# maotian123/loc_lib

Hardware: NVIDIA B200
Metric: registered_points_per_sec (higher is better)
Workload: dtype f64

## Files before the change

loc_lib_b200/csrc/icp_pipeline.cuh:

```cuda
#pragma once
#include "device_utils.cuh"
#include "icp_point.cuh"
#include "knn_warp.cuh"

namespace locreg {

struct DevResult {
    int iters, updates, converged, degenerate;
    long long n_effective, n_inlier;
    double sum_sq_res;
    int pose_written, pad_;
};
static_assert(sizeof(DevResult) == 48, "DevResult must match locreg_result");

struct AlignState {
    double pose[7];
    DevResult res;
    int stop;
    int pad;
};

constexpr int kTile = 256;
constexpr unsigned int kNoNeighbour = kNoPos;

// ... 104 lines not shown
    if (threadIdx.x == 0) tile_begin[S] = carry;
}

__global__ void k_tile_table(BatchView bv, unsigned int n_tiles, TileRec* tiles) {
    const unsigned int t = blockIdx.x * blockDim.x + threadIdx.x;
    if (t >= n_tiles) return;
    bv.tiles = nullptr;
    const TileCoord c = locate_tile_thread(bv, t);
    TileRec r;
    r.scan = c.scan; r.first = c.first; r.count = c.valid ? c.count : 0u; r.valid = c.valid ? 1u : 0u;
    r.base = c.src_base; r.pad = 0;
    tiles[t] = r;
}

#ifndef LR_NN_MIN_BLOCKS
#define LR_NN_MIN_BLOCKS 6
#endif
constexpr int kNnSeeds = 1, kNnTwoPass = 2;
struct RingQueue {
    unsigned int* count;
    uint2* entries;
};

__device__ __forceinline__ void tile_queue_append(bool mine, unsigned int row, unsigned int scan, unsigned int* pending,
                                                  unsigned int* done, unsigned int* staged, const RingQueue& queue,
                                                  unsigned int* local_rows = nullptr, unsigned int* local_n = nullptr) {
    const unsigned int lane = threadIdx.x & 31, n_warps = blockDim.x >> 5;
#if defined(LR_APPEND_BARRIER)
    if (mine) staged[atomicAdd(pending, 1u)] = row;
    __syncthreads();
    if (threadIdx.x >= 32) return;
    (void)done; (void)n_warps;
    {
        const unsigned int n = *pending;
        if (n == 0u) return;
        if (local_rows != nullptr) {
            for (unsigned int i = lane; i < n; i += 32) local_rows[i] = staged[i];
            if (lane == 0) { *local_n = n; atomicAdd(queue.count, n); }
            return;
        }
        unsigned int base = 0;
        if (lane == 0) base = atomicAdd(queue.count, n);
        base = __shfl_sync(0xffffffffu, base, 0);
        for (unsigned int i = lane; i < n; i += 32) queue.entries[base + i] = make_uint2(staged[i], scan);
        return;
    }
#endif
    if (mine) staged[atomicAdd(pending, 1u)] = row;
    __syncwarp();
    unsigned int last = 0;
    if (lane == 0) {
        __threadfence_block();
        last = atomicAdd(done, 1u) == n_warps - 1 ? 1u : 0u;
        __threadfence_block();
    }
    if (!__shfl_sync(0xffffffffu, last, 0)) return;
    __syncwarp();
    const unsigned int n = *reinterpret_cast<volatile unsigned int*>(pending);
    if (n == 0u) return;
    if (local_rows != nullptr) {
        for (unsigned int i = lane; i < n; i += 32) local_rows[i] = reinterpret_cast<volatile unsigned int*>(staged)[i];
        if (lane == 0) { *local_n = n; atomicAdd(queue.count, n); }
        return;
    }
    unsigned int base = 0;
    if (lane == 0) base = atomicAdd(queue.count, n);
    base = __shfl_sync(0xffffffffu, base, 0);
    for (unsigned int i = lane; i < n; i += 32)
        queue.entries[base + i] = make_uint2(reinterpret_cast<volatile unsigned int*>(staged)[i], scan);
}

constexpr int kNnTrack = 4;
constexpr int kNnFirstTrack = 16;
constexpr int kNnFused = 8;
#ifndef LR_NN_TRACK_MIN_BLOCKS
#define LR_NN_TRACK_MIN_BLOCKS LR_NN_MIN_BLOCKS
#endif
template <int K, bool TRACKED>
__device__ __forceinline__ void icp_nn_tile(unsigned int tile, const VoxelMapView& map, const BatchView& bv,
                                            const AlignState* __restrict__ states, int ignore_stop, int mode,
                                            unsigned int* __restrict__ nn_pos, unsigned char* __restrict__ plane_valid, KnnTrack* track,
                                            const RingQueue& queue, unsigned int* local_rows = nullptr, unsigned int* local_n = nullptr) {
    __shared__ Pose T;
    const TileCoord tc = locate_tile(bv, tile);
    if (!tc.valid) return;
    const AlignState* st = states + tc.scan;
    if (st->stop && !ignore_stop) return;
    if (threadIdx.x == 0) pose_load(T, st->pose);
    __shared__ unsigned int blk_pending, blk_done, blk_scan;
    __shared__ unsigned int staged[kTile];
    __shared__ unsigned char scan_list[kTile];
    if (threadIdx.x == 0) { blk_pending = 0u; blk_done = 0u; blk_scan = 0u; }
// ... 49 lines not shown
        const float qx = static_cast<float>(wx), qy = static_cast<float>(wy), qz = static_cast<float>(wz);
        if (tracked) done = knn_query_fast_track<K>(map, qx, qy, qz, nn, seeds, tr);
        else done = knn_query_fast<K>(map, qx, qy, qz, nn, seeds, (mode & kNnTwoPass) != 0);
        same = done && (mode & kNnSeeds) != 0;
        same = same && knn_same_set<K>(seeds, nn.pos);
    }
    if (in_tile) {
#pragma unroll
        for (int j = 0; j < K; ++j) out[j] = nn.pos[j];
        if (plane_valid && !same) plane_valid[row] = 0;
        if (track) track[row] = tr;
    }
    tile_queue_append(!done, static_cast<unsigned int>(row), tc.scan, &blk_pending, &blk_done, staged, queue, local_rows, local_n);
}
template <int K, bool TRACKED>
__global__ void __launch_bounds__(kTile, TRACKED ? LR_NN_TRACK_MIN_BLOCKS : LR_NN_MIN_BLOCKS) k_icp_nn(VoxelMapView map, BatchView bv,
                                                                    const AlignState* __restrict__ states, int ignore_stop,
                                                                    int mode, unsigned int* __restrict__ nn_pos,
                                                                    unsigned char* __restrict__ plane_valid, KnnTrack* track,
                                                                    RingQueue queue) {
    icp_nn_tile<K, TRACKED>(blockIdx.x, map, bv, states, ignore_stop, mode, nn_pos, plane_valid, track, queue);
}

#ifndef LR_FINISH_MIN_BLOCKS
#define LR_FINISH_MIN_BLOCKS 8
#endif
template <int K>
__global__ void __launch_bounds__(128, LR_FINISH_MIN_BLOCKS) k_icp_nn_finish(VoxelMapView map, CoarseLevels coarse, BatchView bv,
                                                       const AlignState* __restrict__ states, unsigned int* __restrict__ nn_pos,
                                                       KnnTrack* track, RingQueue queue, unsigned int min_count, unsigned int max_count) {
    const unsigned int n = *queue.count;
    if (n < min_count || n >= max_count) return;
    const unsigned int lane = threadIdx.x & 31;
    while (true) {
        unsigned int base = 0;
        if (lane == 0) base = atomicAdd(queue.count + 1, 32u);
        base = __shfl_sync(0xffffffffu, base, 0);
        if (base >= n) break;
        const unsigned int e = base + lane;
        if (e >= n) continue;
        const uint2 q = queue.entries[e];
        const size_t src_idx = bv.offsets ? static_cast<size_t>(q.x) : static_cast<size_t>(q.x) - static_cast<size_t>(q.y) * bv.n_single;
        const float4 sp = bv.src[src_idx];
        Pose T;
        pose_load(T, states[q.y].pose);
        double wx, wy, wz;
// ... 28 lines not shown
    const float4 sp = bv.src[src_idx];
    Pose T;
    pose_load(T, states[q.y].pose);
    double wx, wy, wz;
    pose_apply(T, static_cast<double>(sp.x), static_cast<double>(sp.y), static_cast<double>(sp.z), wx, wy, wz);
    qx = static_cast<float>(wx); qy = static_cast<float>(wy); qz = static_cast<float>(wz);
}
__global__ void __launch_bounds__(256) k_queue_bin_count(BatchView bv, const AlignState* __restrict__ states, RingQueue queue,
                                                         unsigned int min_count, float inv_bin, unsigned int bucket_mask, int sub_bits,
                                                         unsigned int* __restrict__ bucket_of, unsigned int* hist) {
    const unsigned int n = *queue.count;
    if (n < min_count) return;
    for (unsigned int e = blockIdx.x * blockDim.x + threadIdx.x; e < n; e += gridDim.x * blockDim.x) {
        float qx, qy, qz;
        queue_entry_query(queue.entries[e], bv, states, qx, qy, qz);
        const int bx = cell_of(cell_coord_f(qx, inv_bin)), by = cell_of(cell_coord_f(qy, inv_bin)), bz = cell_of(cell_coord_f(qz, inv_bin));
        const unsigned long long key = pack_cell(bx >> sub_bits, by >> sub_bits, bz >> sub_bits);
        unsigned int mort = 0u;
        for (int j = 0; j < sub_bits; ++j)
            mort |= (((static_cast<unsigned int>(bx) >> j) & 1u) << (3 * j)) | (((static_cast<unsigned int>(by) >> j) & 1u) << (3 * j + 1)) |
                    (((static_cast<unsigned int>(bz) >> j) & 1u) << (3 * j + 2));
        const unsigned int b = ((hash_block(key) << (3 * sub_bits)) | mort) & bucket_mask;
        bucket_of[e] = b;
        atomicAdd(&hist[b], 1u);
    }
}
__global__ void __launch_bounds__(256) k_queue_bin_scatter(RingQueue queue, unsigned int min_count, const unsigned int* __restrict__ bucket_of,
                                                           unsigned int* cursor, uint2* __restrict__ sorted) {
    const unsigned int n = *queue.count;
    if (n < min_count) return;
    for (unsigned int e = blockIdx.x * blockDim.x + threadIdx.x; e < n; e += gridDim.x * blockDim.x)
        sorted[atomicAdd(&cursor[bucket_of[e]], 1u)] = queue.entries[e];
}

#ifndef LR_PYR_MIN_BLOCKS
#define LR_PYR_MIN_BLOCKS 8
#endif
#ifndef LR_PYR_REFILL
#define LR_PYR_REFILL 8
#endif
template <int K>
__global__ void __launch_bounds__(128, LR_PYR_MIN_BLOCKS) k_icp_nn_pyr(VoxelMapView map, const __grid_constant__ PyrView py, BatchView bv,
                                                    const AlignState* __restrict__ states, unsigned int* __restrict__ nn_pos,
                                                    KnnTrack* track, RingQueue queue, unsigned int min_count) {
    const unsigned int n = *queue.count;
    if (n < min_count) return;
    const unsigned int lane = threadIdx.x & 31;
    PyrWalk<K> w;
    unsigned long long todo[kPyrStack];
    constexpr int kFree = 4, kDead = 5;
    int st = kFree, bit = 0;
    bool exhausted = false;
    unsigned int row = 0;
    while (true) {
        const unsigned int b_node = __ballot_sync(0xffffffffu, st == kPyrNode), b_point = __ballot_sync(0xffffffffu, st == kPyrPoint),
// ... 540 lines not shown
```

loc_lib_b200/csrc/icp_staged.cuh:

```cuda
#pragma once
#include "icp_pipeline.cuh"

namespace locreg {

#ifndef LR_STAGE_CAP
#define LR_STAGE_CAP 2048
#endif
constexpr unsigned int kStageCap = LR_STAGE_CAP;
constexpr unsigned int kStageTab = 512;

template <int K>
struct KnnSel {
    float d[K];
    unsigned int p[K];
    float d6;
};
template <int K>
__device__ __forceinline__ void sel_init(KnnSel<K>& s) {
#pragma unroll
    for (int j = 0; j < K; ++j) { s.d[j] = INFINITY; s.p[j] = kNoPos; }
    s.d6 = INFINITY;
}
template <int K>
__device__ __forceinline__ void sel_push(KnnSel<K>& s, float d, unsigned int p) {
// ... 9 lines not shown
}
template <int K>
__device__ __forceinline__ bool sel_unambiguous(const KnnSel<K>& s) {
    bool ok = !(s.d[K - 1] == s.d6);
#pragma unroll
    for (int j = 0; j + 1 < K; ++j) ok = ok && !(s.d[j] == s.d[j + 1] && s.p[j + 1] != kNoPos);
    return ok;
}

LR_HD void knn_find_list_key(const VoxelMapView& m, unsigned long long key, unsigned int& beg, unsigned int& cnt) {
    unsigned int h = hash_block(key) & m.nbr_mask;
    beg = 0; cnt = 0;
    while (true) {
        const NbrSlot s = m.nbr_slots[h];
        if (s.key == key) { beg = s.start; cnt = s.count; return; }
        if (s.key == kEmptyKey) return;
        h = (h + 1) & m.nbr_mask;
    }
}

#ifndef LR_STAGED_MIN_BLOCKS
#define LR_STAGED_MIN_BLOCKS 4
#endif
template <int K, int MODE>
__global__ void __launch_bounds__(kTile, LR_STAGED_MIN_BLOCKS)
k_icp_nn_staged(VoxelMapView map, BatchView bv, const AlignState* __restrict__ states, int ignore_stop, unsigned int* __restrict__ nn_pos,
                unsigned char* __restrict__ plane_valid, KnnTrack* track, RingQueue queue) {
    __shared__ Pose T;
    __shared__ float4 s_cand[kStageCap];
    __shared__ unsigned long long s_key[kStageTab];
    __shared__ unsigned short s_slot_id[kStageTab];
    __shared__ unsigned long long s_lkey[kTile];
    __shared__ unsigned int s_beg[kTile], s_cnt[kTile];
    __shared__ unsigned int s_off[kTile + 1];
    __shared__ unsigned int s_nlists;
    __shared__ unsigned int blk_pending, blk_done;
    __shared__ unsigned int staged[kTile];
    const TileCoord tc = locate_tile(bv, blockIdx.x);
    if (!tc.valid) return;
    const AlignState* st = states + tc.scan;
    if (st->stop && !ignore_stop) return;
    if (threadIdx.x == 0) {
        pose_load(T, st->pose);
        blk_pending = 0u; blk_done = 0u; s_nlists = 0u;
    }
    for (unsigned int i = threadIdx.x; i < kStageTab; i += kTile) s_key[i] = kEmptyKey;
    const bool in_tile = threadIdx.x < tc.count;
    const unsigned int p = tc.first + (in_tile ? threadIdx.x : 0u);
    const float4 sp = bv.src[tc.src_base + p];
    const size_t row = static_cast<size_t>(tc.out_base + p);
    unsigned int* out = nn_pos + row * K;
    unsigned int seeds[K];
#pragma unroll
    for (int j = 0; j < K; ++j) seeds[j] = (MODE != 0 && in_tile) ? out[j] : kNoPos;
    __syncthreads();
    const bool valid = in_tile && finite3(sp.x, sp.y, sp.z) && map.n_pts != 0;
    float qx = 0.0f, qy = 0.0f, qz = 0.0f;
    KnnCellFrame c{};
    bool listed = false;
    unsigned int my_slot = 0;
    if (valid) {
        double wx, wy, wz;
        pose_apply(T, static_cast<double>(sp.x), static_cast<double>(sp.y), static_cast<double>(sp.z), wx, wy, wz);
        qx = static_cast<float>(wx); qy = static_cast<float>(wy); qz = static_cast<float>(wz);
        c = knn_frame(map, qx, qy, qz);
        listed = c.R0 == 1;
        if (listed) {
            const unsigned long long key = pack_cell(c.fx, c.fy, c.fz);
            unsigned int h = hash_block(key) & (kStageTab - 1);
            while (true) {
                const unsigned long long prev = atomicCAS(&s_key[h], kEmptyKey, key);
                if (prev == kEmptyKey) {
                    const unsigned int id = atomicAdd(&s_nlists, 1u);
                    s_slot_id[h] = static_cast<unsigned short>(id);
                    s_lkey[id] = key;
                    break;
                }
                if (prev == key) break;
                h = (h + 1) & (kStageTab - 1);
            }
            my_slot = h;
        }
    }
    KnnResult<K> res;
    knn_init(res);
    float4 sd[K];
// ... 92 lines not shown
        }
        if (sel_unambiguous(sel)) {
#pragma unroll
            for (int j = 0; j < K; ++j) { res.d2[j] = sel.d[j]; res.pos[j] = sel.p[j]; }
        } else {
            knn_init(res);
            knn_seed<K>(map, qx, qy, qz, seeds, res);
            sel.d6 = INFINITY;
            if (listed) {
                const float4* lst = off < kStageCap ? s_cand + off : map.pts + s_beg[id];
                for (unsigned int i = 0; i < cnt; ++i) {
                    const float4 p = lst[i];
                    knn_offer_track(map.pts, res, dis2_f32(qx, qy, qz, p.x, p.y, p.z), static_cast<unsigned int>(float_as_int(p.w)), sel.d6);
                }
            }
        }
        if (listed) {
            done = knn_list_final<K>(map, c, res);
            if (MODE == 2 && done) tr.margin = knn_track_margin<K>(map, c, res, sel.d6, qx, qy, qz);
        }
        same = done && MODE != 0;
        same = same && knn_same_set<K>(seeds, res.pos);
    }
    if (in_tile) {
#pragma unroll
        for (int j = 0; j < K; ++j) out[j] = res.pos[j];
        if (plane_valid && !same) plane_valid[row] = 0;
        if (track) track[row] = tr;
    }
    tile_queue_append(!done, static_cast<unsigned int>(row), tc.scan, &blk_pending, &blk_done, staged, queue);
}

}
```

loc_lib_b200/csrc/locreg.cu:

```cuda
#include "../../include/locreg.h"

#include <algorithm>
#include <cstdio>
#include <cstdlib>
#include <cstring>
#include <string>
#include <deque>
#include <vector>

#include "align_kernels.cuh"
#include "device_map.cuh"
#include "device_inc_ndt.cuh"
#include "device_ndt.cuh"
#include "filters.cuh"
#include "icp_fused.cuh"
#include "icp_staged.cuh"
#include "icp_persist.cuh"
#include "reloc_select.cuh"
#include "nccl_dyn.h"

#include <nvtx3/nvToolsExt.h>

using namespace locreg;

// ... 57 lines not shown
    std::vector<cudaStream_t> chunk_streams;
    std::vector<cudaEvent_t> chunk_done;
    cudaEvent_t loam_ev[2] = {nullptr, nullptr};
    DeviceVoxelMap icp_map;
    DeviceVoxelMap icp_coarse[kCoarseLevels];
    DeviceVoxelMap icp_mid;
    CoarseLevels coarse_views(int mid_shells = -1, int coarse_shells = -1) const {
        CoarseLevels c{};
        c.mid_shells_p1 = mid_shells + 1;
        c.coarse_shells_p1 = coarse_shells + 1;
        for (int l = 0; l < kCoarseLevels; ++l) c.lv[l] = icp_coarse[l].view();
        c.mid = icp_mid.view();
        c.pyr = icp_map.pyramid();
        c.pyr_mode = 0;
        return c;
    }
    DeviceNdtMap ndt_map;
    DeviceIncNdtMap inc_ndt_map;
    bool has_target = false;
    ncclComm_t comm = nullptr;
    int comm_rank = 0, comm_world = 1;
    DevBuf d_gather_pose, d_gather_res, d_bcast;
    DevBuf d_raw, d_src4, d_out, d_partials, d_state, d_acc, d_gate, d_nn, d_offsets, d_poses_in, d_poses_out, d_results,
        d_scores, d_misc, d_target, d_nnpos, d_tile_begin, d_tiles, d_states, d_ringq, d_ringc, d_sortq, d_sortb, d_sorth, d_rescanq, d_rescanc, d_loam, d_lmap_new, d_global, d_local, d_same, d_plane, d_pstat, d_track;
    DevBuf d_stage_keys, d_stage_slot, d_stage_idx, d_stage_poses, d_stage_scores, d_stage_rounds, d_stage_sel;
    size_t n_global = 0, global_stride = 0;
    struct KeyFrame { void* p = nullptr; size_t n = 0; };
    std::deque<KeyFrame> keyframes;
    DevBuf d_lmap, d_lmap_tmp;
    size_t n_lmap = 0, lmap_stride = 0;
    void clear_keyframes() {
        for (KeyFrame& k : keyframes) if (k.p) cudaFree(k.p);
        keyframes.clear();
        n_lmap = 0; lmap_stride = 0;
    }
    PinBuf h_in, h_out, h_small;
    double last_ms = 0;
    long long last_launches = 0;
    bool profile = false;
    std::vector<cudaEvent_t> prof_events;
    std::vector<int> prof_class;
    double prof_ms[4] = {0, 0, 0, 0};
    long long prof_launches[4] = {0, 0, 0, 0};
    std::vector<float> prof_trace;

    IcpParams icp_params() const {
        IcpParams p;
        p.max_nn_distance = opt.max_nn_distance;
        p.max_plane_distance = opt.max_plane_distance;
        p.max_line_distance = opt.max_line_distance;
        p.plane_fit_eps = 1e-2;
        p.eps = opt.eps;
        p.max_iteration = opt.max_iteration;
        p.min_effective_pts = opt.min_effective_pts;
        return p;
    }
    NdtParams ndt_params() const {
        NdtParams p;
        p.res_outlier_th = opt.res_outlier_th;
        p.eps = opt.eps;
        p.max_iteration = opt.max_iteration;
        p.min_effective_pts = opt.min_effective_pts;
        p.min_pts_in_voxel = opt.min_pts_in_voxel;
        p.n_nearby = opt.nearby_type == LOCREG_NEARBY6 ? 7 : 1;
        return p;
    }
// ... 137 lines not shown
}
void prof_collect(locreg_handle* h) {
    if (!h->profile) return;
    LR_CUDA(cudaStreamSynchronize(h->stream));
    for (size_t i = 0; i + 1 < h->prof_events.size(); i += 2) {
        float ms = 0;
        LR_CUDA(cudaEventElapsedTime(&ms, h->prof_events[i], h->prof_events[i + 1]));
        const int c = h->prof_class[i / 2];
        h->prof_ms[c] += ms;
        h->prof_launches[c] += 1;
        if (getenv("LOCREG_PROFILE_TRACE")) fprintf(stderr, "locreg-trace class %d %.4f ms\n", c, ms);
    }
    for (cudaEvent_t e : h->prof_events) cudaEventDestroy(e);
    h->prof_events.clear();
    h->prof_class.clear();
}

struct IcpJob {
    BatchView bv{};
    AlignState* states = nullptr;
    unsigned int n_tiles = 0;
    size_t n_scratch_points = 0;
    size_t partials_off = 0, ringc_off = 0, ringq_off = 0;
};

template <int METHOD>
const double* icp_launch_eval(locreg_handle* h, const IcpJob& job, int ignore_stop, int nn_mode, unsigned char* gate, int* nn_idx) {
    constexpr int K = METHOD == kIcpP2P ? 1 : 5;
    const VoxelMapView map = h->icp_map.view();
    h->d_nnpos.reserve(job.n_scratch_points * K * sizeof(unsigned int));
    h->d_ringq.reserve(job.n_scratch_points * sizeof(uint2));
    h->d_track.reserve(job.n_scratch_points * sizeof(KnnTrack));
    const bool small = job.n_tiles <= 2u * static_cast<unsigned int>(h->num_sms);
    const bool cache = METHOD == kIcpP2Plane;
    if (cache) {
        h->d_same.reserve(job.n_scratch_points);
        h->d_plane.reserve(job.n_scratch_points * 4 * sizeof(double));
        h->d_pstat.reserve(job.n_scratch_points);
    }
    h->d_partials.reserve((job.partials_off + 2 * static_cast<size_t>(job.n_tiles) * kPartialDoubles) * sizeof(double));
    h->d_ringc.reserve((job.ringc_off + 2) * sizeof(unsigned int));
    unsigned int* const ringc = h->d_ringc.as<unsigned int>() + job.ringc_off;
    double* const partials_a = h->d_partials.as<double>() + job.partials_off;
    if (!(nn_mode & kNnSeeds)) LR_CUDA(cudaMemsetAsync(ringc, 0, 2 * sizeof(unsigned int), h->stream));
    if (job.n_tiles == 0) return nullptr;
    const RingQueue queue{ringc, h->d_ringq.as<uint2>() + job.ringq_off};
    static const int fused_on = getenv("LOCREG_FUSED") ? atoi(getenv("LOCREG_FUSED")) : 0;
    const bool fused = METHOD == kIcpP2Plane && (nn_mode & kNnFused) && !gate && !nn_idx && fused_on;
    double* partials_b = partials_a + static_cast<size_t>(job.n_tiles) * kPartialDoubles;
    static const int staged_on = getenv("LOCREG_STAGED") ? atoi(getenv("LOCREG_STAGED")) : 1;
    int staged_mode = -1;
    if (map.nbr_slots != nullptr) {
        if (nn_mode == kNnTwoPass && (staged_on & 1)) staged_mode = 0;
        else if (nn_mode == kNnSeeds && (staged_on & 2)) staged_mode = 1;
        else if ((nn_mode & kNnTrack) && (nn_mode & kNnFirstTrack) && (staged_on & 4)) staged_mode = 2;
    }
    prof_mark(h, 0, true);
    if (fused)
    {
        h->d_rescanq.reserve(job.n_scratch_points * sizeof(uint2));
        h->d_rescanc.reserve(2 * sizeof(unsigned int));
        const RingQueue rescan{h->d_rescanc.as<unsigned int>(), h->d_rescanq.as<uint2>()};
        LR_CUDA(cudaMemsetAsync(h->d_rescanc.p, 0, 2 * sizeof(unsigned int), h->stream));
        LR_LAUNCH(k_icp_track_p2plane, job.n_tiles, kTile, 0, h->stream, map, h->icp_params(), job.bv, job.states, ignore_stop,
                  h->d_track.as<KnnTrack>(), rescan, h->d_plane.as<double>(), h->d_pstat.as<unsigned char>(), partials_a);
        const unsigned int g = static_cast<unsigned int>(std::min<size_t>((job.n_scratch_points + 127) / 128, static_cast<size_t>(h->num_sms) * 8));
        LR_LAUNCH(k_icp_rescan, g, 128, 0, h->stream, map, job.bv, job.states, h->d_nnpos.as<unsigned int>(), h->d_same.as<unsigned char>(),
                  h->d_track.as<KnnTrack>(), queue, rescan);
    }
    else if (staged_mode >= 0) {
        unsigned char* pv = cache ? h->d_same.as<unsigned char>() : nullptr;
        if (staged_mode == 0)
            LR_LAUNCH((k_icp_nn_staged<K, 0>), job.n_tiles, kTile, 0, h->stream, map, job.bv, job.states, ignore_stop, h->d_nnpos.as<unsigned int>(), pv, h->d_track.as<KnnTrack>(), queue);
        else if (staged_mode == 1)
            LR_LAUNCH((k_icp_nn_staged<K, 1>), job.n_tiles, kTile, 0, h->stream, map, job.bv, job.states, ignore_stop, h->d_nnpos.as<unsigned int>(), pv, h->d_track.as<KnnTrack>(), queue);
        else
            LR_LAUNCH((k_icp_nn_staged<K, 2>), job.n_tiles, kTile, 0, h->stream, map, job.bv, job.states, ignore_stop, h->d_nnpos.as<unsigned int>(), pv, h->d_track.as<KnnTrack>(), queue);
    } else if (nn_mode & kNnTrack)
        LR_LAUNCH((k_icp_nn<K, true>), job.n_tiles, kTile, 0, h->stream, map, job.bv, job.states, ignore_stop, nn_mode, h->d_nnpos.as<unsigned int>(),
                  cache ? h->d_same.as<unsigned char>() : nullptr, h->d_track.as<KnnTrack>(), queue);
    else
        LR_LAUNCH((k_icp_nn<K, false>), job.n_tiles, kTile, 0, h->stream, map, job.bv, job.states, ignore_stop, nn_mode, h->d_nnpos.as<unsigned int>(),
                  cache ? h->d_same.as<unsigned char>() : nullptr, h->d_track.as<KnnTrack>(), queue);
    prof_mark(h, 0, false);
    prof_mark(h, 3, true);
    constexpr unsigned int kWarpFinishMax = 16384;
    static const int track_env = getenv("LOCREG_TRACK") ? atoi(getenv("LOCREG_TRACK")) : 1;
    KnnTrack* stage2_track = track_env ? h->d_track.as<KnnTrack>() : nullptr;
    static const int sort_on = getenv("LOCREG_SORT") ? atoi(getenv("LOCREG_SORT")) : 1;
    static const int sort_batch = getenv("LOCREG_SORT_BATCH") ? atoi(getenv("LOCREG_SORT_BATCH")) : 0;
    static const double sort_frac = getenv("LOCREG_SORT_FRAC") ? atof(getenv("LOCREG_SORT_FRAC")) : 0.1;
    static const double sort_bin = getenv("LOCREG_SORT_BIN") ? atof(getenv("LOCREG_SORT_BIN")) : 1.0;
    static const int sort_bits = getenv("LOCREG_SORT_BITS") ? atoi(getenv("LOCREG_SORT_BITS")) : 24;
    static const int sort_sub = getenv("LOCREG_SORT_SUB") ? std::min(5, std::max(0, atoi(getenv("LOCREG_SORT_SUB")))) : 3;
    static const int pyr_kernel = getenv("LOCREG_PYR_KERNEL") ? atoi(getenv("LOCREG_PYR_KERNEL")) : 0;
    static const unsigned int sort_min = getenv("LOCREG_SORT_MIN") ? static_cast<unsigned int>(std::max(1, atoi(getenv("LOCREG_SORT_MIN")))) : kWarpFinishMax;
    const bool sortable = !small && sort_on && (job.bv.offsets == nullptr || sort_batch) && job.n_scratch_points < 0xFFFFFFFFull;
    unsigned int long_min = 0xFFFFFFFFu;
    if (sortable)
        long_min = static_cast<unsigned int>(std::max<double>(sort_min, std::min<double>(4.0e9, sort_frac * static_cast<double>(job.n_scratch_points))));
    {
        const unsigned int g = static_cast<unsigned int>(std::min<size_t>((job.n_scratch_points + 3) / 4, static_cast<size_t>(h->num_sms) * 8));
        LR_LAUNCH(k_icp_nn_rings<K>, g, 128, 0, h->stream, map, h->coarse_views(), job.bv, job.states, h->d_nnpos.as<unsigned int>(), stage2_track, queue,
                  small ? 0xFFFFFFFFu : std::min(kWarpFinishMax, long_min));
    }
    if (!small) {
        const PyrView pyr = h->icp_map.pyramid();
        RingQueue long_queue = queue;
        if (sortable) {
            const unsigned int buckets = 1u << sort_bits;
            h->d_sortq.reserve(job.n_scratch_points * sizeof(uint2));
            h->d_sortb.reserve(job.n_scratch_points * sizeof(unsigned int));
            h->d_sorth.reserve(static_cast<size_t>(buckets) * sizeof(unsigned int));
            LR_CUDA(cudaMemsetAsync(h->d_sorth.p, 0, static_cast<size_t>(buckets) * sizeof(unsigned int), h->stream));
            const unsigned int gs = static_cast<unsigned int>(std::min<size_t>((job.n_scratch_points + 255) / 256, static_cast<size_t>(h->num_sms) * 8));
            LR_LAUNCH(k_queue_bin_count, gs, 256, 0, h->stream, job.bv, job.states, queue, long_min, static_cast<float>(1.0 / sort_bin), buckets - 1, sort_sub,
                      h->d_sortb.as<unsigned int>(), h->d_sorth.as<unsigned int>());
            exclusive_scan_u32(h->d_sorth.as<unsigned int>(), h->d_sorth.as<unsigned int>(), buckets, nullptr, h->stream);
            LR_LAUNCH(k_queue_bin_scatter, gs, 256, 0, h->stream, queue, long_min, h->d_sortb.as<unsigned int>(), h->d_sorth.as<unsigned int>(),
                      h->d_sortq.as<uint2>());
// ... 34 lines not shown
        LR_LAUNCH(k_icp_fit, (job.n_tiles + group - 1) / group, kTile, 0, h->stream, map, h->icp_params(), job.bv, job.states, ignore_stop,
                  h->d_nnpos.as<unsigned int>(), h->d_same.as<unsigned char>(), h->d_plane.as<double>(), h->d_pstat.as<unsigned char>(), group);
    }
    LR_LAUNCH(k_icp_post<METHOD>, job.n_tiles, kTile, 0, h->stream, map, h->icp_params(), job.bv, job.states, ignore_stop,
              h->d_nnpos.as<unsigned int>(), partials_a, gate, nn_idx, ringc,
              cache ? h->d_plane.as<double>() : nullptr, cache ? h->d_pstat.as<unsigned char>() : nullptr);
    prof_mark(h, 1, false);
    return nullptr;
}
template <int METHOD>
void icp_launch_solve(locreg_handle* h, const IcpJob& job, int mode, double* acc_out, const double* partials_b = nullptr) {
    prof_mark(h, 2, true);
    LR_LAUNCH(k_icp_solve<METHOD>, (job.bv.S + 3) / 4, 128, 0, h->stream, h->icp_params(), job.bv, job.states,
              h->d_partials.as<double>() + job.partials_off, partials_b, mode, acc_out);
    prof_mark(h, 2, false);
}
int icp_loop_nn_mode(int it) {
    static const int tp_iters = getenv("LOCREG_TWOPASS_ITERS") ? atoi(getenv("LOCREG_TWOPASS_ITERS")) : 1;
    static const int track = getenv("LOCREG_TRACK") ? atoi(getenv("LOCREG_TRACK")) : 1;
    static const int track_from = getenv("LOCREG_TRACK_FROM") ? atoi(getenv("LOCREG_TRACK_FROM")) : 3;
    const int seeded = track && it >= track_from ? (kNnSeeds | kNnTrack | (it > track_from ? kNnFused : kNnFirstTrack)) : kNnSeeds;
    return it == 0 ? kNnTwoPass : (it < tp_iters ? (kNnSeeds | kNnTwoPass) : seeded);
}
template <int METHOD>
void icp_run_loop(locreg_handle* h, const IcpJob& job, int final_eval) {
    for (int it = 0; it < h->opt.max_iteration; ++it) {
        const double* pb = icp_launch_eval<METHOD>(h, job, 0, icp_loop_nn_mode(it), nullptr, nullptr);
        icp_launch_solve<METHOD>(h, job, 1, nullptr, pb);
    }
    if (final_eval) {
        const double* pb = icp_launch_eval<METHOD>(h, job, 1, h->opt.max_iteration > 0 ? kNnSeeds : kNnTwoPass, nullptr, nullptr);
        icp_launch_solve<METHOD>(h, job, 0, nullptr, pb);
    }
}
void loam_run_loop(locreg_handle* surf, locreg_handle* edge, const IcpJob& js, const IcpJob& je, int max_iteration,
                   double eps, DevResult* d_half, int final_eval = 0) {
    const auto trip = [&](int ignore_stop, int nn_mode, int mode) {
        LR_CUDA(cudaStreamWaitEvent(edge->stream, surf->loam_ev[0], 0));
        const double* eb = icp_launch_eval<kIcpP2Line>(edge, je, ignore_stop, nn_mode, nullptr, nullptr);
        LR_CUDA(cudaEventRecord(surf->loam_ev[1], edge->stream));
        const double* sb = icp_launch_eval<kIcpP2Plane>(surf, js, ignore_stop, nn_mode, nullptr, nullptr);
        LR_CUDA(cudaStreamWaitEvent(surf->stream, surf->loam_ev[1], 0));
        prof_mark(surf, 2, true);
        LR_LAUNCH(k_loam_solve, (js.bv.S + 3) / 4, 128, 0, surf->stream, js.bv, surf->d_partials.as<double>(), sb,
                  surf->opt.min_effective_pts, je.bv, edge->d_partials.as<double>(), eb, edge->opt.min_effective_pts, js.states,
                  eps, max_iteration, mode, d_half);
        prof_mark(surf, 2, false);
        LR_CUDA(cudaEventRecord(surf->loam_ev[0], surf->stream));
// ... 600 lines not shown
                                 size_t S, const double* poses_out_init) {
    NvtxRange nvtx_r("locreg:align_batch");
    const size_t total = static_cast<size_t>(offsets[S]);
    const float* first = reinterpret_cast<const float*>(reinterpret_cast<const char*>(srcs) + static_cast<size_t>(offsets[0]) * stride);
    const double* poses_out = poses_out_init;
    const size_t base = static_cast<size_t>(offsets[0]);
    const size_t n_pts = total - base;
    const bool pipelined = !is_ndt(h) && S >= 16 && n_pts >= (1u << 20) && is_pinned_or_device(first);
    const float4* src4 = pipelined ? nullptr : stage_cloud(h, first, n_pts, stride, false);
    h->d_offsets.reserve((S + 1) * sizeof(long long));
    h->d_poses_in.reserve(S * 7 * sizeof(double));
    h->d_poses_out.reserve(S * 7 * sizeof(double));
    h->d_results.reserve(S * sizeof(DevResult));
    std::vector<long long> rel(S + 1);
    for (size_t s = 0; s <= S; ++s) rel[s] = offsets[s] - static_cast<long long>(base);
    LR_CUDA(cudaMemcpyAsync(h->d_offsets.p, rel.data(), (S + 1) * sizeof(long long), cudaMemcpyHostToDevice, h->stream));
    LR_CUDA(cudaMemcpyAsync(h->d_poses_in.p, poses_in, S * 7 * sizeof(double), cudaMemcpyHostToDevice, h->stream));
    LR_CUDA(cudaMemcpyAsync(h->d_poses_out.p, poses_out, S * 7 * sizeof(double), cudaMemcpyHostToDevice, h->stream));
    LR_CUDA(cudaStreamSynchronize(h->stream));
    const unsigned int Su = static_cast<unsigned int>(S);
    if (pipelined) {
        static const int streams_env = getenv("LOCREG_CHUNK_STREAMS") ? atoi(getenv("LOCREG_CHUNK_STREAMS")) : 1;
        static const bool fused_env = getenv("LOCREG_FUSED") && atoi(getenv("LOCREG_FUSED")) != 0;
        static const bool sort_batch_env = getenv("LOCREG_SORT_BATCH") && atoi(getenv("LOCREG_SORT_BATCH")) != 0;
        const bool may_run_concurrently = streams_env && !h->profile && !fused_env && !sort_batch_env;
        static const std::vector<double> kEnvWeights = []() {
            std::vector<double> w;
            if (const char* e = getenv("LOCREG_CHUNK_WEIGHTS")) {
                for (const char* p = e; *p;) {
                    char* end = nullptr;
                    const double v = strtod(p, &end);
                    if (end == p) break;
                    if (v > 0.0) w.push_back(v);
                    if (*end != ',') break;
                    p = end + 1;
                }
                if (w.size() > 16) w.resize(16);
            } else if (getenv("LOCREG_CHUNKS") || getenv("LOCREG_CHUNK_RATIO")) {
                const size_t n = getenv("LOCREG_CHUNKS") ? std::max(1, std::min(16, atoi(getenv("LOCREG_CHUNKS")))) : 2;
                const double ratio = getenv("LOCREG_CHUNK_RATIO") ? std::min(16.0, std::max(1.0, atof(getenv("LOCREG_CHUNK_RATIO")))) : 8.0;
                double v = 1.0;
                for (size_t c = 0; c < n; ++c, v *= ratio) w.push_back(v);
            }
            return w;
        }();
        static const std::vector<double> kConcurrentWeights{1.0, 2.0, 3.0, 3.0}, kSerialWeights{1.0, 8.0}, kHugeWeights{1.0, 3.0, 9.0, 27.0, 41.0};
        const std::vector<double>& kWeights = !kEnvWeights.empty() ? kEnvWeights
                                              : !may_run_concurrently || n_pts < (4u << 20) ? kSerialWeights
// ... 12 lines not shown
        double total_w = 0.0, acc_w = 0.0;
        for (size_t c = 0; c < kChunks; ++c) total_w += kWeights[c];
        for (size_t c = 1; c < kChunks; ++c) {
            acc_w += kWeights[c - 1];
            const long long want = static_cast<long long>(static_cast<double>(n_pts) * acc_w / total_w);
            size_t s = std::lower_bound(rel.begin(), rel.end(), want) - rel.begin();
            s = std::min(std::max(s, cut.back()), S);
            cut.push_back(s);
        }
        cut.push_back(S);
        for (size_t c = 0; c < kChunks; ++c) {
            const size_t p0 = static_cast<size_t>(rel[cut[c]]), p1 = static_cast<size_t>(rel[cut[c + 1]]);
            if (p1 > p0)
                LR_CUDA(cudaMemcpyAsync(h->d_raw.as<unsigned char>() + p0 * stride, reinterpret_cast<const char*>(first) + p0 * stride,
                                        (p1 - p0) * stride, cudaMemcpyHostToDevice, h->copy_stream));
            LR_CUDA(cudaEventRecord(h->chunk_events[c], h->copy_stream));
        }
        const bool concurrent = may_run_concurrently && kChunks > 1;
        std::vector<size_t> tile_off(kChunks + 1, 0);
        for (size_t c = 0; c < kChunks; ++c) {
            const size_t pts = static_cast<size_t>(rel[cut[c + 1]] - rel[cut[c]]);
            tile_off[c + 1] = tile_off[c] + pts / kTile + (cut[c + 1] - cut[c]);
        }
        if (concurrent) {
            const size_t K5 = h->opt.method == LOCREG_ICP_P2P ? 1 : 5;
            h->d_partials.reserve(2 * tile_off[kChunks] * kPartialDoubles * sizeof(double));
            h->d_tiles.reserve(tile_off[kChunks] * sizeof(TileRec));
            h->d_tile_begin.reserve((S + kChunks) * sizeof(unsigned int));
            h->d_ringc.reserve(2 * kChunks * sizeof(unsigned int));
            h->d_nnpos.reserve(n_pts * K5 * sizeof(unsigned int));
            h->d_ringq.reserve(n_pts * sizeof(uint2));
            h->d_track.reserve(n_pts * sizeof(KnnTrack));
            if (h->opt.method == LOCREG_ICP_P2PLANE) {
                h->d_same.reserve(n_pts);
                h->d_plane.reserve(n_pts * 4 * sizeof(double));
                h->d_pstat.reserve(n_pts);
            }
            while (h->chunk_streams.size() + 1 < kChunks) {
                cudaStream_t st;
                LR_CUDA(cudaStreamCreateWithFlags(&st, cudaStreamNonBlocking));
                h->chunk_streams.push_back(st);
                cudaEvent_t e;
                LR_CUDA(cudaEventCreateWithFlags(&e, cudaEventDisableTiming));
                h->chunk_done.push_back(e);
            }
        }
        h->begin_timing();
        cudaStream_t const main_stream = h->stream;
        for (size_t c = 0; c < kChunks; ++c) {
            const size_t s0 = cut[c], s1 = cut[c + 1];
            if (concurrent && c > 0) h->stream = h->chunk_streams[c - 1];
            struct Restore { locreg_handle* h; cudaStream_t s; ~Restore() { h->stream = s; } } restore{h, main_stream};
            LR_CUDA(cudaStreamWaitEvent(h->stream, h->chunk_events[c], 0));
            if (s1 > s0) {
                const size_t p0 = static_cast<size_t>(rel[s0]), p1 = static_cast<size_t>(rel[s1]);
                const unsigned int Sc = static_cast<unsigned int>(s1 - s0);
                if (stride != 16 && p1 > p0) {
                    const unsigned int grid = static_cast<unsigned int>(std::min<size_t>((p1 - p0 + 255) / 256, 4096));
                    LR_LAUNCH(k_pack_float4, grid, 256, 0, h->stream, h->d_raw.as<unsigned char>() + p0 * stride, p1 - p0, stride,
                              h->d_src4.as<float4>() + p0);
                }
                const float4* all4 = stride == 16 ? h->d_raw.as<float4>() : h->d_src4.as<float4>();
                IcpJob job = icp_batch_job(h, all4, h->d_offsets.as<long long>() + s0, Sc, p1 - p0, concurrent ? tile_off[c] : 0,
                                           concurrent ? s0 + c : 0);
                job.states = h->d_states.as<AlignState>() + s0;
                job.n_scratch_points = n_pts;
                if (concurrent) {
                    job.partials_off = 2 * tile_off[c] * kPartialDoubles;
                    job.ringc_off = 2 * c;
                    job.ringq_off = p0;
                }
                LR_LAUNCH(k_states_init, (Sc + 255) / 256, 256, 0, h->stream, h->d_poses_in.as<double>() + s0 * 7, Sc, h->opt.max_iteration, h->opt.zero_initial_translation, job.states);
                ICP_DISPATCH(h, icp_run_loop<M>(h, job, 0));
                LR_LAUNCH(k_states_export, (Sc + 255) / 256, 256, 0, h->stream, job.states, Sc, h->d_poses_out.as<double>() + s0 * 7,
                          h->d_results.as<DevResult>() + s0);
            }
            if (concurrent && c > 0) {
                LR_CUDA(cudaEventRecord(h->chunk_done[c - 1], h->stream));
                LR_CUDA(cudaStreamWaitEvent(main_stream, h->chunk_done[c - 1], 0));
            }
        }
        h->end_timing();
    } else {
        h->begin_timing();
        if (is_ndt(h)) {
            NDT_DISPATCH(h, ndt_run_batch(h, PB, src4, h->d_offsets.as<long long>(), h->d_poses_in.as<double>(),
                                          h->d_poses_out.as<double>(), h->d_results.as<DevResult>(), Su));
        } else {
            const IcpJob job = icp_batch_job(h, src4, h->d_offsets.as<long long>(), Su, n_pts);
            LR_LAUNCH(k_states_init, (Su + 255) / 256, 256, 0, h->stream, h->d_poses_in.as<double>(), Su, h->opt.max_iteration, h->opt.zero_initial_translation, job.states);
            ICP_DISPATCH(h, icp_run_loop<M>(h, job, 0));
            LR_LAUNCH(k_states_export, (Su + 255) / 256, 256, 0, h->stream, job.states, Su, h->d_poses_out.as<double>(), h->d_results.as<DevResult>());
        }
// ... 659 lines not shown
    if (!h || !nv) return LOCREG_E_ARG;
    *nv = h->opt.method == LOCREG_NDT_INCREMENTAL ? h->inc_ndt_map.size(h->stream) : h->ndt_map.view().n_voxels;
    return LOCREG_OK;
}
int locreg_ndt_get_voxels(locreg_handle* h, int32_t* keys, double* mu, double* info, int32_t* npts) {
    return guarded(h, [&]() {
        std::vector<int> k, c;
        std::vector<double> m, f;
        if (h->opt.method == LOCREG_NDT_INCREMENTAL) h->inc_ndt_map.download(k, m, f, c, h->stream);
        else h->ndt_map.download(k, m, f, c, h->stream);
        if (keys) std::memcpy(keys, k.data(), k.size() * sizeof(int));
        if (mu) std::memcpy(mu, m.data(), m.size() * sizeof(double));
        if (info) std::memcpy(info, f.data(), f.size() * sizeof(double));
        if (npts) std::memcpy(npts, c.data(), c.size() * sizeof(int));
        return LOCREG_OK;
    });
}

int locreg_profile(locreg_handle* h, int32_t enable, double* ms4, int64_t* launches4) {
    return guarded(h, [&]() {
        prof_collect(h);
        if (ms4) for (int i = 0; i < 4; ++i) ms4[i] = h->prof_ms[i];
        if (launches4) for (int i = 0; i < 4; ++i) launches4[i] = h->prof_launches[i];
        for (int i = 0; i < 4; ++i) { h->prof_ms[i] = 0; h->prof_launches[i] = 0; }
        h->profile = enable != 0;
        return LOCREG_OK;
    });
}

int locreg_index_info(locreg_handle* h, size_t* bytes, size_t* points, size_t* lists_or_voxels) {
    if (!h) { g_last_error = "null handle"; return LOCREG_E_ARG; }
    return guarded(h, [&]() {
        size_t b = 0, p = 0, l = 0;
        if (h->opt.method == LOCREG_NDT_DIRECT) {
            b = h->ndt_map.bytes(); l = h->ndt_map.view().n_voxels;
        } else if (h->opt.method == LOCREG_NDT_INCREMENTAL) {
            l = h->inc_ndt_map.size(h->stream);
        } else {
            b = h->icp_map.bytes() + h->icp_mid.bytes();
            for (int i = 0; i < kCoarseLevels; ++i) b += h->icp_coarse[i].bytes();
            p = h->icp_map.view().n_pts;
            l = h->icp_map.n_lists();
        }
        if (bytes) *bytes = b;
        if (points) *points = p;
        if (lists_or_voxels) *lists_or_voxels = l;
        return LOCREG_OK;
// ... 11 lines not shown
```

Baseline: 829.2 million.

## Spatially sort batched scan points once before ICP loop for staged NN

Before the ICP iterations of a batched job, all points are filled into an entry list, binned by their transformed world-cell with a hash-plus-Morton key, and scattered into a spatially ordered slot list. The first-pass staged NN kernel then runs over these sorted slots, with each thread loading its own scan's pose, so nearby queries share tiles and staged candidate lists. Separately, an optional warp-aggregated atomic path is added to the bin-count and scatter kernels. The sort costs extra launches and memory, and its order is based on the initial poses, so it drifts as poses change. Per-thread pose loads also replace the shared per-tile pose.

```diff
diff --git a/loc_lib_b200/csrc/icp_pipeline.cuh b/loc_lib_b200/csrc/icp_pipeline.cuh
--- a/loc_lib_b200/csrc/icp_pipeline.cuh
+++ b/loc_lib_b200/csrc/icp_pipeline.cuh
@@ -150,9 +150,27 @@
     uint2* entries;
 };
 
+struct SlotView {
+    const uint2* ent;
+    const unsigned int* count;
+    unsigned int base;
+};
+__device__ __forceinline__ TileCoord slot_tile(const SlotView& sl, unsigned int t) {
+    TileCoord c{};
+    const unsigned int n = *sl.count;
+    c.valid = static_cast<size_t>(t) * kTile < n;
+    if (c.valid) {
+        c.first = sl.base + t * kTile;
+        c.count = min(static_cast<unsigned int>(kTile), n - t * kTile);
+    }
+    return c;
+}
+
+template <bool SORTED = false>
 __device__ __forceinline__ void tile_queue_append(bool mine, unsigned int row, unsigned int scan, unsigned int* pending,
                                                   unsigned int* done, unsigned int* staged, const RingQueue& queue,
-                                                  unsigned int* local_rows = nullptr, unsigned int* local_n = nullptr) {
+                                                  unsigned int* local_rows = nullptr, unsigned int* local_n = nullptr,
+                                                  const uint2* slot_ent = nullptr) {
     const unsigned int lane = threadIdx.x & 31, n_warps = blockDim.x >> 5;
 #if defined(LR_APPEND_BARRIER)
     if (mine) staged[atomicAdd(pending, 1u)] = row;
@@ -170,7 +188,7 @@
         unsigned int base = 0;
         if (lane == 0) base = atomicAdd(queue.count, n);
         base = __shfl_sync(0xffffffffu, base, 0);
-        for (unsigned int i = lane; i < n; i += 32) queue.entries[base + i] = make_uint2(staged[i], scan);
+        for (unsigned int i = lane; i < n; i += 32) queue.entries[base + i] = SORTED ? slot_ent[staged[i]] : make_uint2(staged[i], scan);
         return;
     }
 #endif
@@ -194,8 +212,10 @@
     unsigned int base = 0;
     if (lane == 0) base = atomicAdd(queue.count, n);
     base = __shfl_sync(0xffffffffu, base, 0);
-    for (unsigned int i = lane; i < n; i += 32)
-        queue.entries[base + i] = make_uint2(reinterpret_cast<volatile unsigned int*>(staged)[i], scan);
+    for (unsigned int i = lane; i < n; i += 32) {
+        const unsigned int r = reinterpret_cast<volatile unsigned int*>(staged)[i];
+        queue.entries[base + i] = SORTED ? slot_ent[r] : make_uint2(r, scan);
+    }
 }
 
 constexpr int kNnTrack = 4;
@@ -291,6 +311,14 @@
     icp_nn_tile<K, TRACKED>(blockIdx.x, map, bv, states, ignore_stop, mode, nn_pos, plane_valid, track, queue);
 }
 
+__global__ void k_order_fill(BatchView bv, uint2* __restrict__ entries, unsigned int* count) {
+    const TileCoord tc = locate_tile(bv, blockIdx.x);
+    if (blockIdx.x == 0 && threadIdx.x == 0) *count = static_cast<unsigned int>(bv.offsets[bv.S] - bv.offsets[0]);
+    if (!tc.valid || threadIdx.x >= tc.count) return;
+    const long long row = tc.out_base + tc.first + threadIdx.x;
+    entries[row - bv.offsets[0]] = make_uint2(static_cast<unsigned int>(row), tc.scan);
+}
+
 #ifndef LR_FINISH_MIN_BLOCKS
 #define LR_FINISH_MIN_BLOCKS 8
 #endif
@@ -365,15 +393,32 @@
                     (((static_cast<unsigned int>(bz) >> j) & 1u) << (3 * j + 2));
         const unsigned int b = ((hash_block(key) << (3 * sub_bits)) | mort) & bucket_mask;
         bucket_of[e] = b;
+#if defined(LR_QUEUE_AGG)
+        const unsigned int peers = __match_any_sync(__activemask(), b);
+        if ((threadIdx.x & 31u) == static_cast<unsigned int>(__ffs(peers) - 1)) atomicAdd(&hist[b], static_cast<unsigned int>(__popc(peers)));
+#else
         atomicAdd(&hist[b], 1u);
+#endif
     }
 }
 __global__ void __launch_bounds__(256) k_queue_bin_scatter(RingQueue queue, unsigned int min_count, const unsigned int* __restrict__ bucket_of,
                                                            unsigned int* cursor, uint2* __restrict__ sorted) {
     const unsigned int n = *queue.count;
     if (n < min_count) return;
+#if defined(LR_QUEUE_AGG)
+    for (unsigned int e = blockIdx.x * blockDim.x + threadIdx.x; e < n; e += gridDim.x * blockDim.x) {
+        const unsigned int b = bucket_of[e];
+        const unsigned int am = __activemask(), peers = __match_any_sync(am, b);
+        const unsigned int lane = threadIdx.x & 31u, leader = static_cast<unsigned int>(__ffs(peers) - 1);
+        unsigned int pos = 0;
+        if (lane == leader) pos = atomicAdd(&cursor[b], static_cast<unsigned int>(__popc(peers)));
+        pos = __shfl_sync(am, pos, leader) + static_cast<unsigned int>(__popc(peers & ((1u << lane) - 1u)));
+        sorted[pos] = queue.entries[e];
+    }
+#else
     for (unsigned int e = blockIdx.x * blockDim.x + threadIdx.x; e < n; e += gridDim.x * blockDim.x)
         sorted[atomicAdd(&cursor[bucket_of[e]], 1u)] = queue.entries[e];
+#endif
 }
 
 #ifndef LR_PYR_MIN_BLOCKS
diff --git a/loc_lib_b200/csrc/icp_staged.cuh b/loc_lib_b200/csrc/icp_staged.cuh
--- a/loc_lib_b200/csrc/icp_staged.cuh
+++ b/loc_lib_b200/csrc/icp_staged.cuh
@@ -55,10 +55,10 @@
 #ifndef LR_STAGED_MIN_BLOCKS
 #define LR_STAGED_MIN_BLOCKS 4
 #endif
-template <int K, int MODE>
-__global__ void __launch_bounds__(kTile, LR_STAGED_MIN_BLOCKS)
-k_icp_nn_staged(VoxelMapView map, BatchView bv, const AlignState* __restrict__ states, int ignore_stop, unsigned int* __restrict__ nn_pos,
-                unsigned char* __restrict__ plane_valid, KnnTrack* track, RingQueue queue) {
+template <int K, int MODE, bool SORTED>
+__device__ __forceinline__ void icp_nn_staged_tile(VoxelMapView map, BatchView bv, const AlignState* __restrict__ states,
+                                                   int ignore_stop, unsigned int* __restrict__ nn_pos, unsigned char* __restrict__ plane_valid,
+                                                   KnnTrack* track, RingQueue queue, SlotView sl) {
     __shared__ Pose T;
     __shared__ float4 s_cand[kStageCap];
     __shared__ unsigned long long s_key[kStageTab];
@@ -69,32 +69,46 @@
     __shared__ unsigned int s_nlists;
     __shared__ unsigned int blk_pending, blk_done;
     __shared__ unsigned int staged[kTile];
-    const TileCoord tc = locate_tile(bv, blockIdx.x);
+    TileCoord tc;
+    if constexpr (SORTED) tc = slot_tile(sl, blockIdx.x);
+    else tc = locate_tile(bv, blockIdx.x);
     if (!tc.valid) return;
     const AlignState* st = states + tc.scan;
-    if (st->stop && !ignore_stop) return;
+    if constexpr (!SORTED) {
+        if (st->stop && !ignore_stop) return;
+    }
     if (threadIdx.x == 0) {
-        pose_load(T, st->pose);
+        if constexpr (!SORTED) pose_load(T, st->pose);
         blk_pending = 0u; blk_done = 0u; s_nlists = 0u;
     }
     for (unsigned int i = threadIdx.x; i < kStageTab; i += kTile) s_key[i] = kEmptyKey;
     const bool in_tile = threadIdx.x < tc.count;
     const unsigned int p = tc.first + (in_tile ? threadIdx.x : 0u);
-    const float4 sp = bv.src[tc.src_base + p];
-    const size_t row = static_cast<size_t>(tc.out_base + p);
+    uint2 ent = make_uint2(0u, 0u);
+    if constexpr (SORTED) ent = sl.ent[p];
+    const float4 sp = bv.src[SORTED ? static_cast<long long>(ent.x) : tc.src_base + p];
+    const size_t row = SORTED ? static_cast<size_t>(ent.x) : static_cast<size_t>(tc.out_base + p);
     unsigned int* out = nn_pos + row * K;
     unsigned int seeds[K];
 #pragma unroll
     for (int j = 0; j < K; ++j) seeds[j] = (MODE != 0 && in_tile) ? out[j] : kNoPos;
-    __syncthreads();
-    const bool valid = in_tile && finite3(sp.x, sp.y, sp.z) && map.n_pts != 0;
+    Pose Tl;
+    bool live = true;
+    if constexpr (SORTED) {
+        const AlignState* s = states + ent.y;
+        live = in_tile && (!s->stop || ignore_stop);
+        if (live) pose_load(Tl, s->pose);
+    }
+    __syncthreads();
+    const bool valid = in_tile && live && finite3(sp.x, sp.y, sp.z) && map.n_pts != 0;
     float qx = 0.0f, qy = 0.0f, qz = 0.0f;
     KnnCellFrame c{};
     bool listed = false;
     unsigned int my_slot = 0;
     if (valid) {
         double wx, wy, wz;
-        pose_apply(T, static_cast<double>(sp.x), static_cast<double>(sp.y), static_cast<double>(sp.z), wx, wy, wz);
+        if constexpr (SORTED) pose_apply(Tl, static_cast<double>(sp.x), static_cast<double>(sp.y), static_cast<double>(sp.z), wx, wy, wz);
+        else pose_apply(T, static_cast<double>(sp.x), static_cast<double>(sp.y), static_cast<double>(sp.z), wx, wy, wz);
         qx = static_cast<float>(wx); qy = static_cast<float>(wy); qz = static_cast<float>(wz);
         c = knn_frame(map, qx, qy, qz);
         listed = c.R0 == 1;
@@ -233,13 +247,26 @@
         same = done && MODE != 0;
         same = same && knn_same_set<K>(seeds, res.pos);
     }
-    if (in_tile) {
+    if (in_tile && live) {
 #pragma unroll
         for (int j = 0; j < K; ++j) out[j] = res.pos[j];
         if (plane_valid && !same) plane_valid[row] = 0;
         if (track) track[row] = tr;
     }
-    tile_queue_append(!done, static_cast<unsigned int>(row), tc.scan, &blk_pending, &blk_done, staged, queue);
-}
-
-}
+    tile_queue_append<SORTED>(!done, SORTED ? p : static_cast<unsigned int>(row), tc.scan, &blk_pending, &blk_done, staged, queue, nullptr,
+                              nullptr, sl.ent);
+}
+template <int K, int MODE>
+__global__ void __launch_bounds__(kTile, LR_STAGED_MIN_BLOCKS)
+k_icp_nn_staged(VoxelMapView map, BatchView bv, const AlignState* __restrict__ states, int ignore_stop, unsigned int* __restrict__ nn_pos,
+                unsigned char* __restrict__ plane_valid, KnnTrack* track, RingQueue queue) {
+    icp_nn_staged_tile<K, MODE, false>(map, bv, states, ignore_stop, nn_pos, plane_valid, track, queue, SlotView{});
+}
+template <int K, int MODE>
+__global__ void __launch_bounds__(kTile, LR_STAGED_MIN_BLOCKS)
+k_icp_nn_staged_sorted(VoxelMapView map, BatchView bv, const AlignState* __restrict__ states, int ignore_stop, unsigned int* __restrict__ nn_pos,
+                       unsigned char* __restrict__ plane_valid, KnnTrack* track, RingQueue queue, SlotView sl) {
+    icp_nn_staged_tile<K, MODE, true>(map, bv, states, ignore_stop, nn_pos, plane_valid, track, queue, sl);
+}
+
+}
diff --git a/loc_lib_b200/csrc/locreg.cu b/loc_lib_b200/csrc/locreg.cu
--- a/loc_lib_b200/csrc/locreg.cu
+++ b/loc_lib_b200/csrc/locreg.cu
@@ -103,7 +103,7 @@
     int comm_rank = 0, comm_world = 1;
     DevBuf d_gather_pose, d_gather_res, d_bcast;
     DevBuf d_raw, d_src4, d_out, d_partials, d_state, d_acc, d_gate, d_nn, d_offsets, d_poses_in, d_poses_out, d_results,
-        d_scores, d_misc, d_target, d_nnpos, d_tile_begin, d_tiles, d_states, d_ringq, d_ringc, d_sortq, d_sortb, d_sorth, d_rescanq, d_rescanc, d_loam, d_lmap_new, d_global, d_local, d_same, d_plane, d_pstat, d_track;
+        d_scores, d_misc, d_target, d_nnpos, d_tile_begin, d_tiles, d_states, d_ringq, d_ringc, d_sortq, d_sortb, d_sorth, d_slot_ent, d_slotc, d_rescanq, d_rescanc, d_loam, d_lmap_new, d_global, d_local, d_same, d_plane, d_pstat, d_track;
     DevBuf d_stage_keys, d_stage_slot, d_stage_idx, d_stage_poses, d_stage_scores, d_stage_rounds, d_stage_sel;
     size_t n_global = 0, global_stride = 0;
     struct KeyFrame { void* p = nullptr; size_t n = 0; };
@@ -121,8 +121,8 @@
     bool profile = false;
     std::vector<cudaEvent_t> prof_events;
     std::vector<int> prof_class;
-    double prof_ms[4] = {0, 0, 0, 0};
-    long long prof_launches[4] = {0, 0, 0, 0};
+    double prof_ms[5] = {0, 0, 0, 0, 0};
+    long long prof_launches[5] = {0, 0, 0, 0, 0};
     std::vector<float> prof_trace;
 
     IcpParams icp_params() const {
@@ -306,8 +306,14 @@
     unsigned int n_tiles = 0;
     size_t n_scratch_points = 0;
     size_t partials_off = 0, ringc_off = 0, ringq_off = 0;
+    SlotView sl{};
+    size_t slotc_off = 0, sorth_off = 0;
 };
 
+int icp_staged_modes() {
+    static const int staged_on = getenv("LOCREG_STAGED") ? atoi(getenv("LOCREG_STAGED")) : 1;
+    return staged_on;
+}
 template <int METHOD>
 const double* icp_launch_eval(locreg_handle* h, const IcpJob& job, int ignore_stop, int nn_mode, unsigned char* gate, int* nn_idx) {
     constexpr int K = METHOD == kIcpP2P ? 1 : 5;
@@ -332,7 +338,7 @@
     static const int fused_on = getenv("LOCREG_FUSED") ? atoi(getenv("LOCREG_FUSED")) : 0;
     const bool fused = METHOD == kIcpP2Plane && (nn_mode & kNnFused) && !gate && !nn_idx && fused_on;
     double* partials_b = partials_a + static_cast<size_t>(job.n_tiles) * kPartialDoubles;
-    static const int staged_on = getenv("LOCREG_STAGED") ? atoi(getenv("LOCREG_STAGED")) : 1;
+    const int staged_on = icp_staged_modes();
     int staged_mode = -1;
     if (map.nbr_slots != nullptr) {
         if (nn_mode == kNnTwoPass && (staged_on & 1)) staged_mode = 0;
@@ -354,7 +360,11 @@
     }
     else if (staged_mode >= 0) {
         unsigned char* pv = cache ? h->d_same.as<unsigned char>() : nullptr;
-        if (staged_mode == 0)
+        if (staged_mode == 0 && job.sl.ent != nullptr) {
+            if constexpr (K == 5)
+                LR_LAUNCH((k_icp_nn_staged_sorted<K, 0>), job.n_tiles, kTile, 0, h->stream, map, job.bv, job.states, ignore_stop, h->d_nnpos.as<unsigned int>(),
+                          pv, h->d_track.as<KnnTrack>(), queue, job.sl);
+        } else if (staged_mode == 0)
             LR_LAUNCH((k_icp_nn_staged<K, 0>), job.n_tiles, kTile, 0, h->stream, map, job.bv, job.states, ignore_stop, h->d_nnpos.as<unsigned int>(), pv, h->d_track.as<KnnTrack>(), queue);
         else if (staged_mode == 1)
             LR_LAUNCH((k_icp_nn_staged<K, 1>), job.n_tiles, kTile, 0, h->stream, map, job.bv, job.states, ignore_stop, h->d_nnpos.as<unsigned int>(), pv, h->d_track.as<KnnTrack>(), queue);
@@ -372,14 +382,13 @@
     static const int track_env = getenv("LOCREG_TRACK") ? atoi(getenv("LOCREG_TRACK")) : 1;
     KnnTrack* stage2_track = track_env ? h->d_track.as<KnnTrack>() : nullptr;
     static const int sort_on = getenv("LOCREG_SORT") ? atoi(getenv("LOCREG_SORT")) : 1;
-    static const int sort_batch = getenv("LOCREG_SORT_BATCH") ? atoi(getenv("LOCREG_SORT_BATCH")) : 0;
     static const double sort_frac = getenv("LOCREG_SORT_FRAC") ? atof(getenv("LOCREG_SORT_FRAC")) : 0.1;
     static const double sort_bin = getenv("LOCREG_SORT_BIN") ? atof(getenv("LOCREG_SORT_BIN")) : 1.0;
     static const int sort_bits = getenv("LOCREG_SORT_BITS") ? atoi(getenv("LOCREG_SORT_BITS")) : 24;
     static const int sort_sub = getenv("LOCREG_SORT_SUB") ? std::min(5, std::max(0, atoi(getenv("LOCREG_SORT_SUB")))) : 3;
     static const int pyr_kernel = getenv("LOCREG_PYR_KERNEL") ? atoi(getenv("LOCREG_PYR_KERNEL")) : 0;
     static const unsigned int sort_min = getenv("LOCREG_SORT_MIN") ? static_cast<unsigned int>(std::max(1, atoi(getenv("LOCREG_SORT_MIN")))) : kWarpFinishMax;
-    const bool sortable = !small && sort_on && (job.bv.offsets == nullptr || sort_batch) && job.n_scratch_points < 0xFFFFFFFFull;
+    const bool sortable = !small && sort_on && job.bv.offsets == nullptr && job.n_scratch_points < 0xFFFFFFFFull;
     unsigned int long_min = 0xFFFFFFFFu;
     if (sortable)
         long_min = static_cast<unsigned int>(std::max<double>(sort_min, std::min<double>(4.0e9, sort_frac * static_cast<double>(job.n_scratch_points))));
@@ -460,8 +469,44 @@
     const int seeded = track && it >= track_from ? (kNnSeeds | kNnTrack | (it > track_from ? kNnFused : kNnFirstTrack)) : kNnSeeds;
     return it == 0 ? kNnTwoPass : (it < tp_iters ? (kNnSeeds | kNnTwoPass) : seeded);
 }
+unsigned int icp_order_bits(size_t n_tiles, size_t n_scratch_points) {
+    const size_t n = std::min(n_tiles * kTile, n_scratch_points);
+    unsigned int b = 10;
+    while (b < 24 && (size_t{1} << b) < n) ++b;
+    return b;
+}
 template <int METHOD>
-void icp_run_loop(locreg_handle* h, const IcpJob& job, int final_eval) {
+void icp_order_job(locreg_handle* h, IcpJob& job) {
+    const bool small = job.n_tiles <= 2u * static_cast<unsigned int>(h->num_sms);
+    if (METHOD != kIcpP2Plane || job.bv.offsets == nullptr || small || h->opt.max_iteration <= 0 || !(icp_staged_modes() & 1) ||
+        h->icp_map.view().nbr_slots == nullptr || job.n_scratch_points >= 0xFFFFFFFFull)
+        return;
+    const size_t n = job.n_scratch_points;
+    const unsigned int buckets = 1u << icp_order_bits(job.n_tiles, n);
+    h->d_ringq.reserve(n * sizeof(uint2));
+    h->d_slot_ent.reserve(n * sizeof(uint2));
+    h->d_sortb.reserve(n * sizeof(unsigned int));
+    h->d_sorth.reserve((job.sorth_off + buckets) * sizeof(unsigned int));
+    h->d_slotc.reserve((job.slotc_off + 1) * sizeof(unsigned int));
+    unsigned int* const count = h->d_slotc.as<unsigned int>() + job.slotc_off;
+    unsigned int* const hist = h->d_sorth.as<unsigned int>() + job.sorth_off;
+    const size_t base = job.ringq_off;
+    const RingQueue entries{count, h->d_ringq.as<uint2>() + base};
+    prof_mark(h, 4, true);
+    LR_LAUNCH(k_order_fill, job.n_tiles, kTile, 0, h->stream, job.bv, entries.entries, count);
+    LR_CUDA(cudaMemsetAsync(hist, 0, static_cast<size_t>(buckets) * sizeof(unsigned int), h->stream));
+    const unsigned int gs = static_cast<unsigned int>(std::min<size_t>((n + 255) / 256, static_cast<size_t>(h->num_sms) * 8));
+    LR_LAUNCH(k_queue_bin_count, gs, 256, 0, h->stream, job.bv, job.states, entries, 0u, h->icp_map.view().inv_cell, buckets - 1, 3,
+              h->d_sortb.as<unsigned int>() + base, hist);
+    exclusive_scan_u32(hist, hist, buckets, nullptr, h->stream);
+    LR_LAUNCH(k_queue_bin_scatter, gs, 256, 0, h->stream, entries, 0u, h->d_sortb.as<unsigned int>() + base, hist, h->d_slot_ent.as<uint2>() + base);
+    prof_mark(h, 4, false);
+    job.sl = SlotView{h->d_slot_ent.as<uint2>(), count, static_cast<unsigned int>(base)};
+}
+template <int METHOD>
+void icp_run_loop(locreg_handle* h, const IcpJob& job_in, int final_eval) {
+    IcpJob job = job_in;
+    icp_order_job<METHOD>(h, job);
     for (int it = 0; it < h->opt.max_iteration; ++it) {
         const double* pb = icp_launch_eval<METHOD>(h, job, 0, icp_loop_nn_mode(it), nullptr, nullptr);
         icp_launch_solve<METHOD>(h, job, 1, nullptr, pb);
@@ -1108,8 +1153,7 @@
     if (pipelined) {
         static const int streams_env = getenv("LOCREG_CHUNK_STREAMS") ? atoi(getenv("LOCREG_CHUNK_STREAMS")) : 1;
         static const bool fused_env = getenv("LOCREG_FUSED") && atoi(getenv("LOCREG_FUSED")) != 0;
-        static const bool sort_batch_env = getenv("LOCREG_SORT_BATCH") && atoi(getenv("LOCREG_SORT_BATCH")) != 0;
-        const bool may_run_concurrently = streams_env && !h->profile && !fused_env && !sort_batch_env;
+        const bool may_run_concurrently = streams_env && !h->profile && !fused_env;
         static const std::vector<double> kEnvWeights = []() {
             std::vector<double> w;
             if (const char* e = getenv("LOCREG_CHUNK_WEIGHTS")) {
@@ -1168,6 +1212,7 @@
             const size_t pts = static_cast<size_t>(rel[cut[c + 1]] - rel[cut[c]]);
             tile_off[c + 1] = tile_off[c] + pts / kTile + (cut[c + 1] - cut[c]);
         }
+        std::vector<size_t> sorth_off(kChunks, 0);
         if (concurrent) {
             const size_t K5 = h->opt.method == LOCREG_ICP_P2P ? 1 : 5;
             h->d_partials.reserve(2 * tile_off[kChunks] * kPartialDoubles * sizeof(double));
@@ -1181,6 +1226,15 @@
                 h->d_same.reserve(n_pts);
                 h->d_plane.reserve(n_pts * 4 * sizeof(double));
                 h->d_pstat.reserve(n_pts);
+                h->d_slot_ent.reserve(n_pts * sizeof(uint2));
+                h->d_sortb.reserve(n_pts * sizeof(unsigned int));
+                h->d_slotc.reserve(kChunks * sizeof(unsigned int));
+                size_t buckets = 0;
+                for (size_t c = 0; c < kChunks; ++c) {
+                    sorth_off[c] = buckets;
+                    buckets += size_t{1} << icp_order_bits(tile_off[c + 1] - tile_off[c], n_pts);
+                }
+                h->d_sorth.reserve(buckets * sizeof(unsigned int));
             }
             while (h->chunk_streams.size() + 1 < kChunks) {
                 cudaStream_t st;
@@ -1215,6 +1269,8 @@
                     job.partials_off = 2 * tile_off[c] * kPartialDoubles;
                     job.ringc_off = 2 * c;
                     job.ringq_off = p0;
+                    job.slotc_off = c;
+                    job.sorth_off = sorth_off[c];
                 }
                 LR_LAUNCH(k_states_init, (Sc + 255) / 256, 256, 0, h->stream, h->d_poses_in.as<double>() + s0 * 7, Sc, h->opt.max_iteration, h->opt.zero_initial_translation, job.states);
                 ICP_DISPATCH(h, icp_run_loop<M>(h, job, 0));
@@ -1920,7 +1976,7 @@
         prof_collect(h);
         if (ms4) for (int i = 0; i < 4; ++i) ms4[i] = h->prof_ms[i];
         if (launches4) for (int i = 0; i < 4; ++i) launches4[i] = h->prof_launches[i];
-        for (int i = 0; i < 4; ++i) { h->prof_ms[i] = 0; h->prof_launches[i] = 0; }
+        for (int i = 0; i < 5; ++i) { h->prof_ms[i] = 0; h->prof_launches[i] = 0; }
         h->profile = enable != 0;
         return LOCREG_OK;
     });
```

Result: no change. 832.9 million, median of 6 (+0.4%).
